# mariaalfaroc/omr_a2s_multimodal_transformer

Hardware: AMD Instinct MI355X
Metric: training samples/sec (higher is better)
Workload: dtype bf16; 1 GPU; C2: image encoder (CNN) + 6-layer d_model=256 kern decoder, fwd+bwd+Adam, dropout on, teacher-forcing noise on; one sample = one score image + its token sequence; per_gpu_batch=32, global_batch=32, image=256x2048x1, seq_len=512, layers=6, d_model=256, vocab=6997, parallelism=dp1

## Files before the change

include/omr_hip.h:

```cpp
#ifndef OMR_HIP_H
#define OMR_HIP_H
#ifdef __cplusplus
extern "C" {
#endif

#define OMR_DTYPE_F32 0
#define OMR_DTYPE_BF16 1
#define OMR_DTYPE_U8 2

int omr_abi_version(void);

int omr_cast(const void* src, int src_dtype, void* dst, int dst_dtype, long n, void* stream);
int omr_add(int dtype, const void* a, const void* b, void* out, long n, void* stream);
int omr_relu_bwd(int dtype, const void* dy, const void* y, void* dx, long n, float scale, void* stream);
int omr_dropout(int dtype, const void* x, void* out, long n, float p, unsigned long long seed, int channel_mode, long per_sample, int C,
                void* stream);
int omr_embed_pe_fwd(int dtype, const long* tokens, const void* table, const float* pe, void* out, long M, int T_len, int d, int vocab,
                     void* stream);
int omr_embed_bwd(int dtype, const long* tokens, const void* dout, float* dtable, long M, int d, int pad_idx, int vocab, void* stream);
int omr_add_pe2d(int dtype, const void* x, const float* pe_hwc, void* out, int B, int h, int w, int C, int maxh, int maxw, void* stream);
int omr_colsum(int dtype, const void* dy, float* db, long M, int N, long ld, void* stream);
int omr_adam(float* p, const float* g, float* m, float* v, void* p_bf16, long n, int step, float lr, float b1, float b2, float eps,
             float grad_scale, void* stream);
int omr_argmax(const float* x, int rows, int n, long ld, long* idx_out, float* val_out, void* stream);
// ... 54 lines not shown
                               const OmrAugment* aug, int dst_dtype, void* out, int B, int H, int W, float pad_value, void* stream);

int omr_gemm(int dtype, int c_dtype, int transA, int transB, int M, int N, int K, const void* A, long lda, const void* B, long ldb, void* C,
             long ldc, const float* bias, int relu, int accumulate, int split_k, float* colsum_a, float drop_p,
             unsigned long long drop_seed, int row_group, int row_group_stride, int row_group_base, int row_group_operand, void* stream);

int omr_quantize_rows_fp8(int dtype, const void* x, long ldx, unsigned char* q, long ldq, float* scale, int M, int K, void* stream);
int omr_gemm_fp8(int c_dtype, int M, int N, int K, const unsigned char* A8, long lda, const float* scale_a, const unsigned char* W8, long ldb,
                 const float* scale_w, void* C, long ldc, const float* bias, int relu, void* stream);

typedef struct omr_dw_problem {
    const void* dy; const void* x; float* dw; float* db;
    int rows, n_out, n_in, row_group; long ld_dy, ld_x, ld_dw; int row_group_stride, row_group_base;
} omr_dw_problem;
int omr_linear_wgrad_grouped(int dtype, int nprob, const omr_dw_problem* problems, void* stream);

int omr_conv3x3_stat_slots(int B, int Ho, int Wo);
int omr_instnorm_reduce_sums(void* workspace, int slots, int B, int C, void* stream);
int omr_conv3x3_fwd(int dtype, const void* x, const void* w, const float* bias, void* y, const float* in_mean, const float* in_rstd,
                    const void* out_mask, float mask_scale, int B, int H, int W, int CIN, int COUT, int stride_h, int stride_w, int dil_h,
                    int dil_w, int Ho, int Wo, int relu, float drop_p, unsigned long long drop_seed, int drop_channel_mode,
                    int stat_mode, double* stat_ws, int stat_slots, const void* stat_x, const float* stat_mean, const float* stat_rstd,
                    void* stream);
int omr_conv3x3_weight_flip(int dtype, const void* w, void* wd, int COUT, int CIN, void* stream);
typedef struct omr_flip_desc { const void* w; void* wd; int cout, cin; } omr_flip_desc;
int omr_conv3x3_weight_flip_grouped(int dtype, int n, const omr_flip_desc* descs, void* stream);
int omr_conv3x3_wgrad(int dtype, const void* x, const void* dy, float* dw, float* db, const float* in_mean, const float* in_rstd, int B, int H, int W,
                      int CIN, int COUT, int stride_h, int stride_w, int Ho, int Wo, void* stream);
int omr_conv3x3_bwd_fused(const void* g, const void* x, const void* w_flipped, void* dx, float* dw, float* db, int B, int H, int W, int CIN,
                          int COUT, int mask_input, float mask_scale, const void* norm_y, const float* norm_mean, const float* norm_rstd,
                          const void* norm_workspace, int norm_slots, int relu_mask, float relu_scale, const float* x_mean, const float* x_rstd,
                          void* stat_workspace, int stat_slots, void* stream);
int omr_conv3x3_bwd_fused_s2(const void* g, const void* x, const void* w_flipped, void* dx, float* dw, float* db, int B, int H, int W,
                             const float* x_mean, const float* x_rstd, void* stat_workspace, int stat_slots, void* stream);
int omr_dwconv3x3(int dtype, const void* x, const void* w, const float* bias, void* y, const float* in_mean, const float* in_rstd,
                  const void* out_mask, float mask_scale, int B, int H, int W, int C, int flip, void* stream);
int omr_dwconv3x3_wgrad(int dtype, const void* x, const void* dy, float* dw, float* db, const float* in_mean, const float* in_rstd, int B,
                        int H, int W, int C, void* stream);

int omr_attn_fwd(int dtype, const void* q, const void* k, const void* v, void* o, float* lse, long ldq, long ldk, long ldv, long ldo,
                 long bsq, long bsk, long bsv, long bso, int B, int H, int T, int S, int head_dim, int causal, int window,
                 const float* key_bias, const int* blk_lq, const int* blk_lkv, float dropout_p, unsigned long long seed,
                 const unsigned long long* drop_words, void* stream);
long omr_attn_dropout_words_count(int B, int H, int T, int S);
int omr_attn_dropout_words(unsigned long long* words, int B, int H, int T, int S, float dropout_p, unsigned long long seed, void* stream);
long omr_attn_workspace_floats(int B, int H, int T, int S, int head_dim, int causal, int backward);
// ... 207 lines not shown
```

omr_a2s_multimodal_transformer_amd/csrc/conv.hip:

```cpp
#include <type_traits>

#include "omr_common.h"
#include "omr_hip.h"

#include "conv3x3_mfma.h"
#include "conv_wgrad.h"
#include "conv1.h"

using omr_conv::ConvArgs;
using omr_conv::TW;
int omr_conv3x3_dispatch_bf16(const ConvArgs& a, hipStream_t s);
int omr_conv3x3_dispatch_f32(const ConvArgs& a, hipStream_t s);

namespace {

constexpr int FLIP_MAX = 32;
struct FlipTable { const void* w[FLIP_MAX]; void* wd[FLIP_MAX]; int cout[FLIP_MAX]; int cin[FLIP_MAX]; };
template <typename T>
__global__ void weight_flip_grouped_kernel(FlipTable t) {
    const int g = blockIdx.y, COUT = t.cout[g], CIN = t.cin[g];
    const T* __restrict__ w = (const T*)t.w[g];
    T* __restrict__ wd = (T*)t.wd[g];
    const long total = (long)COUT * 9 * CIN;
    for (long i = blockIdx.x * (long)blockDim.x + threadIdx.x; i < total; i += (long)gridDim.x * blockDim.x) {
// ... 175 lines not shown
    int gx = (OMR_NUM_CU * occv + gy - 1) / gy; if (gx < 1) gx = 1; if (gx > ntiles) gx = ntiles;
    hipLaunchKernelGGL(kern, dim3(gx, gy), dim3(256), shm, s, a);
    OMR_CHECK_LAUNCH();
    return OMR_OK;
}

template <typename T, int TH, int SH, int SW> int launch_wgrad2(const WgradArgs& a, hipStream_t s) {
    if (a.COUT > 32 && a.CIN > 32) return launch_wgrad3<T, TH, 64, 64, SH, SW>(a, s);
    if (a.COUT > 32) return launch_wgrad3<T, TH, 64, 32, SH, SW>(a, s);
    return launch_wgrad3<T, TH, 32, 32, SH, SW>(a, s);
}

template <typename T, int TH1, int TH2> int launch_wgrad(const WgradArgs& a, hipStream_t s) {
    if (a.sh == 1 && a.sw == 1) return launch_wgrad2<T, TH1, 1, 1>(a, s);
    if (a.sh == 2 && a.sw == 2) return launch_wgrad2<T, TH2, 2, 2>(a, s);
    if (a.sh == 2 && a.sw == 1) return launch_wgrad2<T, TH2, 2, 1>(a, s);
    return OMR_ERR_UNSUPPORTED;
}

inline int ew_grid(long n) { long g = (n + 255) / 256; return (int)(g < 1 ? 1 : (g > 4096 ? 4096 : g)); }

}

extern "C" int omr_conv3x3_fwd(int dtype, const void* x, const void* w, const float* bias, void* y, const float* in_mean, const float* in_rstd,
                               const void* out_mask, float mask_scale, int B, int H, int W, int CIN, int COUT, int stride_h, int stride_w,
                               int dil_h, int dil_w, int Ho, int Wo, int relu, float drop_p, unsigned long long drop_seed,
                               int drop_channel_mode, int stat_mode, double* stat_ws, int stat_slots, const void* stat_x,
                               const float* stat_mean, const float* stat_rstd, void* stream) {
    if (B <= 0 || H <= 0 || W <= 0 || CIN <= 0 || COUT <= 0 || !x || !w || (!y && stat_mode != 4)) return OMR_ERR_ARG;
    if (stride_h < 1 || stride_w < 1 || dil_h < 1 || dil_w < 1 || dil_h > 2 || dil_w > 2) return OMR_ERR_ARG;
    if ((stride_h > 1 || stride_w > 1) && (dil_h > 1 || dil_w > 1)) return OMR_ERR_UNSUPPORTED;
    hipStream_t s = (hipStream_t)stream;
    if (drop_p < 0.f || drop_p >= 1.f || stat_mode < 0 || stat_mode == 3 || stat_mode > 5) return OMR_ERR_ARG;
    if (stat_mode && (!stat_ws || stat_slots < 1)) return OMR_ERR_ARG;
    if (stat_mode >= 2 && (!stat_x || !stat_mean || !stat_rstd)) return OMR_ERR_ARG;
    if (stat_mode >= 4 && (out_mask || bias || drop_p > 0.f)) return OMR_ERR_ARG;
    if (CIN == 1) {
        if (drop_p > 0.f || stat_mode) return OMR_ERR_UNSUPPORTED;
        if (dil_h != 1 || dil_w != 1 || stride_h != 1 || stride_w != 1 || in_mean || out_mask || Ho != H || Wo != W) return OMR_ERR_UNSUPPORTED;
        return omr_conv1_fwd(dtype, x, w, bias, y, B, H, W, COUT, relu, s);
    }
    ConvArgs a;
    a.x = x; a.w = w; a.bias = bias; a.y = y; a.mean = in_mean; a.rstd = in_rstd; a.mask = out_mask; a.mask_scale = mask_scale;
    a.B = B; a.Hr = H; a.Wr = W; a.CIN = CIN; a.Ho = Ho; a.Wo = Wo; a.COUT = COUT;
    a.sh = stride_h; a.sw = stride_w; a.dh = dil_h; a.dw = dil_w; a.relu = relu; a.tiles_w = a.tiles_h = 0;
    a.drop_thresh = OMR_DROP_THRESH16(drop_p); a.drop_scale = 1.f / (1.f - drop_p); a.drop_seed = drop_seed;
    a.drop_channel = drop_channel_mode;
    a.stat_mode = stat_mode; a.stat_ws = stat_ws; a.stat_x = stat_x; a.stat_mean = stat_mean; a.stat_rstd = stat_rstd; a.stat_slots = stat_slots;
    a.stat_relu = 0; a.stat_relu_scale = 1.f;
    if (stat_mode >= 4) { a.stat_relu = relu; a.stat_relu_scale = mask_scale; a.relu = 0; a.mask_scale = 1.f; }
    if (dtype == OMR_BF16) return omr_conv3x3_dispatch_bf16(a, s);
    if (dtype == OMR_F32) return omr_conv3x3_dispatch_f32(a, s);
    return OMR_ERR_UNSUPPORTED;
}

extern "C" int omr_conv3x3_stat_slots(int B, int Ho, int Wo) {
    if (B <= 0 || Ho <= 0 || Wo <= 0) return OMR_ERR_ARG;
    const long tiles = (long)cdiv(Ho, 4) * cdiv(Wo, TW), slots = ((long)OMR_NUM_CU * 8 + B - 1) / B;
    return (int)(tiles < slots ? tiles : slots);
}

extern "C" int omr_conv3x3_weight_flip(int dtype, const void* w, void* wd, int COUT, int CIN, void* stream) {
    if (COUT <= 0 || CIN <= 0) return OMR_ERR_ARG;
    FlipTable t = {};
    t.w[0] = w; t.wd[0] = wd; t.cout[0] = COUT; t.cin[0] = CIN;
    DISPATCH_T(dtype, hipLaunchKernelGGL((weight_flip_grouped_kernel<T>), ew_grid((long)COUT * 9 * CIN), 256, 0, (hipStream_t)stream, t));
    OMR_CHECK_LAUNCH();
    return OMR_OK;
}

extern "C" int omr_conv3x3_weight_flip_grouped(int dtype, int n, const omr_flip_desc* descs, void* stream) {
    if (n < 0 || (n && !descs)) return OMR_ERR_ARG;
// ... 41 lines not shown
```

omr_a2s_multimodal_transformer_amd/csrc/conv3x3_mfma.h:

```cpp
#pragma once
#include <type_traits>

#include "omr_common.h"
#include "launch_setup.h"
#include "instnorm_slots.h"

namespace omr_conv {

constexpr int NORM_MAX = 128;
constexpr int TW = 32;

template <int G, typename F, typename LoadFn, typename StoreFn>
__device__ __forceinline__ void staged_walk(int pix0, int npix, int DP, int il0, int jl0, int di, int dj, int IW, LoadFn load, StoreFn store) {
    int il = il0, jl = jl0;
    for (int base = pix0; base < npix; base += G * DP) {
        F v[G];
        int pix = base;
#pragma unroll
        for (int g = 0; g < G; ++g) {
            if (pix < npix) v[g] = load(il, jl);
            jl += dj; il += di;
            if (jl >= IW) { jl -= IW; ++il; }
            pix += DP;
        }
        pix = base;
#pragma unroll
        for (int g = 0; g < G; ++g) {
            if (pix < npix) store(pix, v[g]);
            pix += DP;
        }
    }
}

__host__ __device__ constexpr bool conv_subpix(int SH, int SW, int DH, int DW, int RPW) { return DH == 2 && DW == 2 && SH == 1 && SW == 1 && RPW == 2; }
__host__ __device__ constexpr int conv_halo_h(int TH, int SH, bool subpix) { return subpix ? ((TH - 1) * SH + 3 + 1) / 2 : (TH - 1) * SH + 3; }
__host__ __device__ constexpr int conv_halo_w(int SW, bool subpix) { return subpix ? ((TW - 1) * SW + 3) / 2 : (TW - 1) * SW + 3; }

struct ConvArgs {
    const void* x; const void* w; const float* bias; void* y;
    const float* mean; const float* rstd;
    const void* mask; float mask_scale;
    int B, Hr, Wr, CIN, Ho, Wo, COUT;
    int sh, sw, dh, dw, relu, tiles_w, tiles_h;
    uint32_t drop_thresh; float drop_scale; uint64_t drop_seed; int drop_channel;
    int stat_mode; double* stat_ws; const void* stat_x; const float* stat_mean; const float* stat_rstd; int stat_slots;
    int stat_relu; float stat_relu_scale;
};

template <typename T, int NT, int RPW, int CK, int SH, int SW, int DH, int DW, bool SINGLE, int EPI>
__global__ __launch_bounds__(256, (SINGLE && NT == 32) ? ((CK == 16 && EPI != 2) ? 4 : 3) : 2) void conv3x3_mfma_kernel(ConvArgs a) {
    typedef typename Frag<T>::type F;
    typedef __attribute__((ext_vector_type(4))) T T4;
    constexpr int VEC = Frag<T>::N;
    constexpr int CKP = CK + VEC;
    constexpr int NB = NT / 32;
    constexpr int TH = 4 * RPW;
    constexpr bool SUBPIX = conv_subpix(SH, SW, DH, DW, RPW);
    constexpr int IH = conv_halo_h(TH, SH, SUBPIX), IW = conv_halo_w(SW, SUBPIX), NPIX = IH * IW;
    constexpr int CPP = CK / VEC;
    constexpr int OP = NT + VEC;
    constexpr int XS_ELEMS = (SINGLE && TH * TW * OP > NPIX * CKP) ? TH * TW * OP : NPIX * CKP;
    extern __shared__ __attribute__((aligned(16))) unsigned char smem_raw[];
    T* Xs = reinterpret_cast<T*>(smem_raw);
    T* Os = Xs;
    T* Ws = Xs + XS_ELEMS;

    const int tid = threadIdx.x, lane = tid & 63, wave = tid >> 6;
    const int n0 = blockIdx.y * NT;
    const int Hv = (a.Hr - 1) * DH + 1, Wv = (a.Wr - 1) * DW + 1;
    const T* W = (const T*)a.w;
    constexpr bool single = SINGLE;
    const int frow = lane & 31, fk = (lane >> 5) * VEC, hsel = 4 * (lane >> 5);
    const int sp_rp = wave >> 1;
    const int sp_row = (wave & 1) * 4 + sp_rp + 2 * (frow >> 4), sp_col = 2 * (frow & 15);

    auto stage_weights = [&](int c0) {
        constexpr int NCH = NT * 9 * CPP, ROUNDS = (NCH + 255) / 256, GB = 4;
#pragma unroll
        for (int r0 = 0; r0 < ROUNDS; r0 += GB) {
            F v[GB];
#pragma unroll
            for (int g = 0; g < GB; ++g) {
                const int c = tid + (r0 + g) * 256, row = c / CPP, kc = (c % CPP) * VEC, n = n0 + row / 9;
                v[g] = frag_zero<T>();
                if (r0 + g < ROUNDS && c < NCH && n < a.COUT) v[g] = *reinterpret_cast<const F*>(W + ((long)n * 9 + row % 9) * a.CIN + c0 + kc);
            }
#pragma unroll
            for (int g = 0; g < GB; ++g) {
                const int c = tid + (r0 + g) * 256, row = c / CPP, kc = (c % CPP) * VEC;
                if (r0 + g < ROUNDS && c < NCH) *reinterpret_cast<F*>(Ws + (long)row * CKP + kc) = v[g];
            }
        }
    };

    __shared__ __attribute__((aligned(16))) float sbias[NT];
    for (int i = tid; i < NT; i += 256) sbias[i] = (a.bias && n0 + i < a.COUT) ? a.bias[n0 + i] : 0.f;

    __shared__ __attribute__((aligned(16))) float snorm[2 * NORM_MAX];
    if (a.mean)
        for (int i = tid; i < a.CIN; i += 256) {
            snorm[i] = a.mean[(long)blockIdx.z * a.CIN + i];
            snorm[NORM_MAX + i] = a.rstd[(long)blockIdx.z * a.CIN + i];
        }

    if (single) stage_weights(0);

    constexpr int CPO = NT / VEC;
    constexpr int NSV = EPI ? VEC : 1;
    float ssum[NSV], ssq[NSV], smu[EPI == 2 ? VEC : 1], srs[EPI == 2 ? VEC : 1];
#pragma unroll
    for (int e = 0; e < NSV; ++e) ssum[e] = ssq[e] = 0.f;
#pragma unroll
    for (int e = 0; e < (EPI == 2 ? VEC : 1); ++e) { smu[e] = 0.f; srs[e] = 1.f; }
    constexpr bool FWD = EPI == 1 || EPI == 3, DROP = EPI == 3;
    const bool stat1 = FWD && a.stat_mode == 1, stat2 = EPI == 2 && (a.stat_mode == 2 || a.stat_mode == 4);
    const bool apply5 = EPI == 2 && a.stat_mode == 5, store_y = a.stat_mode != 4;
    auto flush_stats = [&](int bimg) {
        if constexpr (EPI != 0) {
            constexpr int NGRP = 256 / CPO;
            constexpr int RP = NT + 1;
            static_assert((size_t)NGRP * RP * sizeof(float) <= ((size_t)XS_ELEMS + (size_t)NT * 9 * CKP) * sizeof(T), "reduction scratch fits in the (dead) halo + weight tiles");
            float* red = reinterpret_cast<float*>(smem_raw);
#pragma unroll
            for (int k = 0; k < 2; ++k) {
                __syncthreads();
                const int kcs = (tid % CPO) * VEC, grp = tid / CPO;
#pragma unroll
                for (int e = 0; e < NSV; ++e) red[grp * RP + kcs + e] = k ? ssq[e] : ssum[e];
                __syncthreads();
                for (int i = tid; i < NT; i += 256) {
                    const int n = n0 + i;
                    double acc2 = 0.0;
                    for (int g = 0; g < NGRP; ++g) acc2 += (double)red[g * RP + i];
                    if (n < a.COUT) slot_store(a.stat_ws, bimg, a.stat_slots, a.COUT, n, k, acc2);
                }
            }
        }
    };

    const int tiles_per_img = a.tiles_h * a.tiles_w;
    const int b = blockIdx.z;
    if constexpr (EPI == 2) {
        if (stat2 || apply5) {
            const double* compact = a.stat_ws + slot_compact_offset(a.B, a.stat_slots, a.COUT);
            const double inv_hw = 1.0 / ((double)a.Ho * a.Wo);
#pragma unroll
            for (int e = 0; e < VEC; ++e) {
                const int n = n0 + (tid % CPO) * VEC + e;
                smu[e] = n < a.COUT ? a.stat_mean[(long)b * a.COUT + n] : 0.f;
                srs[e] = n < a.COUT ? a.stat_rstd[(long)b * a.COUT + n] : 1.f;
                if (apply5) {
                    ssum[e] = n < a.COUT ? (float)(compact[((long)b * a.COUT + n) * 2] * inv_hw) : 0.f;
                    ssq[e] = n < a.COUT ? (float)(compact[((long)b * a.COUT + n) * 2 + 1] * inv_hw) : 0.f;
                }
            }
        }
    }
    uint32_t ckeep[NB];
#pragma unroll
    for (int j = 0; j < NB; ++j) ckeep[j] = 0xffffu;
    if constexpr (DROP) {
        if (a.drop_thresh && a.drop_channel) {
#pragma unroll
            for (int j = 0; j < NB; ++j) {
                ckeep[j] = 0;
#pragma unroll
                for (int r = 0; r < 16; r += 2) {
                    const uint32_t hsh = drop_pair_bits(a.drop_seed, ((uint64_t)b * a.COUT + n0 + j * 32 + 8 * (r >> 2) + hsel + (r & 3)) >> 1);
                    ckeep[j] |= (uint32_t)((hsh & 0xffffu) >= a.drop_thresh) << r | (uint32_t)((hsh >> 16) >= a.drop_thresh) << (r + 1);
                }
            }
        }
    }
    constexpr bool PF = true;
    constexpr int XR = (NPIX + 255) / 256;
    constexpr int WNCH = NT * 9 * CPP, WR = SINGLE ? 1 : (WNCH + 255) / 256;
    F xv[XR][CPP], wv[WR];
    unsigned xok = 0;
    const T* X = (const T*)a.x + (long)b * a.Hr * a.Wr * a.CIN;
    auto load_x = [&](int rem, int c0) {
        const int th = rem / a.tiles_w, tw = rem - th * a.tiles_w;
        const int vh0 = th * TH * SH - 1, vw0 = tw * TW * SW - 1;
        xok = 0;
#pragma unroll
        for (int r = 0; r < XR; ++r) {
            const int pix = tid + r * 256;
            const int il = pix / IW, jl = pix - il * IW;
            const int vh = vh0 + (SUBPIX ? 2 * il + 1 : il), vw = vw0 + (SUBPIX ? 2 * jl + 1 : jl);
            const bool ok = pix < NPIX && vh >= 0 && vh < Hv && vw >= 0 && vw < Wv && (vh & (DH - 1)) == 0 && (vw & (DW - 1)) == 0;
            const T* src = X + ((long)(vh >> (DH >> 1)) * a.Wr + (vw >> (DW >> 1))) * a.CIN + c0;
#pragma unroll
            for (int k = 0; k < CPP; ++k) {
                xv[r][k] = frag_zero<T>();
                if (ok) xv[r][k] = *reinterpret_cast<const F*>(src + k * VEC);
            }
            xok |= (unsigned)ok << r;
        }
    };
    auto store_x = [&](int c0) {
#pragma unroll
        for (int r = 0; r < XR; ++r) {
            const int pix = tid + r * 256;
            if (a.mean && ((xok >> r) & 1)) {
#pragma unroll
                for (int k = 0; k < CPP; ++k)
#pragma unroll
                    for (int q4 = 0; q4 < VEC / 4; ++q4) {
                        const f32x4 mu = *reinterpret_cast<const f32x4*>(&snorm[c0 + k * VEC + 4 * q4]);
                        const f32x4 rs = *reinterpret_cast<const f32x4*>(&snorm[NORM_MAX + c0 + k * VEC + 4 * q4]);
#pragma unroll
                        for (int e = 0; e < 4; ++e)
                            xv[r][k][4 * q4 + e] = from_f32<T>((to_f32(xv[r][k][4 * q4 + e]) - mu[e]) * rs[e]);
                    }
            }
            if (pix < NPIX)
#pragma unroll
                for (int k = 0; k < CPP; ++k) *reinterpret_cast<F*>(Xs + (long)pix * CKP + k * VEC) = xv[r][k];
        }
    };
    auto load_w = [&](int c0) {
#pragma unroll
        for (int r = 0; r < WR; ++r) {
            const int c = tid + r * 256, row = c / CPP, kc = (c % CPP) * VEC, n = n0 + row / 9;
            wv[r] = frag_zero<T>();
            if (c < WNCH && n < a.COUT) wv[r] = *reinterpret_cast<const F*>(W + ((long)n * 9 + row % 9) * a.CIN + c0 + kc);
        }
    };
    auto store_w = [&]() {
#pragma unroll
        for (int r = 0; r < WR; ++r) {
            const int c = tid + r * 256, row = c / CPP, kc = (c % CPP) * VEC;
            if (c < WNCH) *reinterpret_cast<F*>(Ws + (long)row * CKP + kc) = wv[r];
        }
    };
    if constexpr (PF) {
        if ((int)blockIdx.x < tiles_per_img) { load_x(blockIdx.x, 0); load_w(0); }
    }

    for (int rem = blockIdx.x; rem < tiles_per_img; rem += gridDim.x) {
        const int th = rem / a.tiles_w, tw = rem - th * a.tiles_w;
        const int oh0 = th * TH, ow0 = tw * TW;
        const int vh0 = oh0 * SH - 1;

        f32x16 acc[RPW][NB];
#pragma unroll
        for (int i = 0; i < RPW; ++i)
#pragma unroll
            for (int j = 0; j < NB; ++j)
#pragma unroll
                for (int r = 0; r < 16; ++r) acc[i][j][r] = 0.f;

        for (int c0 = 0; c0 < a.CIN; c0 += CK) {
            __syncthreads();
            if constexpr (!PF) load_x(rem, c0);
            store_x(c0);
            if constexpr (!SINGLE) store_w();
            __syncthreads();
            if constexpr (PF) {
                int nc0 = c0 + CK, nrem = rem;
                if (nc0 >= a.CIN) { nc0 = 0; nrem = rem + gridDim.x; }
                if (nrem < tiles_per_img) { load_x(nrem, nc0); load_w(nc0); }
            }
            bool row_live[RPW][3];
#pragma unroll
            for (int i = 0; i < RPW; ++i)
#pragma unroll
                for (int kh = 0; kh < 3; ++kh) row_live[i][kh] = DH == 1 || (((vh0 + (wave * RPW + i) * SH + kh) & (DH - 1)) == 0);
            if constexpr (SUBPIX) {
                const int vw0 = ow0 * SW - 1;
#pragma unroll
                for (int tap = 0; tap < 9; ++tap) {
                    const int kh = tap / 3, kw = tap % 3;
                    if (((vh0 + sp_rp + kh) & 1) != 0) continue;
                    const bool lc[2] = {((vw0 + kw) & 1) == 0, ((vw0 + 1 + kw) & 1) == 0};
#pragma unroll
                    for (int kk = 0; kk < CK; kk += KStep<T>::value) {
                        F af[2], bf[NB];
#pragma unroll
                        for (int cp = 0; cp < 2; ++cp)
                            if (lc[cp]) af[cp] = *reinterpret_cast<const F*>(Xs + (long)(((sp_row + kh) >> 1) * IW + ((sp_col + cp + kw) >> 1)) * CKP + kk + fk);
#pragma unroll
                        for (int j = 0; j < NB; ++j)
                            bf[j] = *reinterpret_cast<const F*>(Ws + (long)((j * 32 + frow) * 9 + tap) * CKP + kk + fk);
#pragma unroll
                        for (int cp = 0; cp < 2; ++cp) {
                            if (!lc[cp]) continue;
#pragma unroll
                            for (int j = 0; j < NB; ++j) mma32(acc[cp][j], bf[j], af[cp]);
                        }
                    }
                }
            } else
#pragma unroll
            for (int tap = 0; tap < 9; ++tap) {
                const int kh = tap / 3, kw = tap % 3;
                bool any_live = false;
#pragma unroll
                for (int i = 0; i < RPW; ++i) any_live = any_live || row_live[i][kh];
                if (!any_live) continue;
#pragma unroll
                for (int kk = 0; kk < CK; kk += KStep<T>::value) {
                    F af[RPW], bf[NB];
#pragma unroll
                    for (int i = 0; i < RPW; ++i) {
                        const int pix = ((wave * RPW + i) * SH + kh) * IW + frow * SW + kw;
                        af[i] = *reinterpret_cast<const F*>(Xs + (long)pix * CKP + kk + fk);
                    }
#pragma unroll
                    for (int j = 0; j < NB; ++j)
                        bf[j] = *reinterpret_cast<const F*>(Ws + (long)((j * 32 + frow) * 9 + tap) * CKP + kk + fk);
#pragma unroll
                    for (int i = 0; i < RPW; ++i) {
                        if (!row_live[i][kh]) continue;
#pragma unroll
                        for (int j = 0; j < NB; ++j) mma32(acc[i][j], bf[j], af[i]);
                    }
                }
            }
        }

        const float oscale = a.mask ? a.mask_scale : 1.f;
        const bool drop_chan = DROP && a.drop_thresh != 0 && a.drop_channel;
        __syncthreads();
#pragma unroll
        for (int j = 0; j < NB; ++j)
#pragma unroll
            for (int i = 0; i < RPW; ++i) {
                T* orow = Os + (long)(SUBPIX ? sp_row * TW + sp_col + i : (wave * RPW + i) * TW + frow) * OP + j * 32 + hsel;
#pragma unroll
                for (int g = 0; g < 4; ++g) {
                    T4 o;
                    const uint32_t k4 = ckeep[j] >> (4 * g);
                    const f32x4 bq = *reinterpret_cast<const f32x4*>(&sbias[j * 32 + 8 * g + hsel]);
#pragma unroll
                    for (int e = 0; e < 4; ++e) {
                        float v = acc[i][j][4 * g + e] + bq[e];
                        if (a.relu) v = fmaxf(v, 0.f);
                        if constexpr (DROP) {
                            if (drop_chan) v = ((k4 >> e) & 1u) ? v * a.drop_scale : 0.f;
                        } else {
                            v *= oscale;
                        }
                        o[e] = from_f32<T>(v);
                    }
                    *reinterpret_cast<T4*>(orow + 8 * g) = o;
                }
            }
        __syncthreads();
        T* Y = (T*)a.y + (long)b * a.Ho * a.Wo * a.COUT;
        const T* Mk = a.mask ? (const T*)a.mask + (long)b * a.Ho * a.Wo * a.COUT : nullptr;
        const T* SX = (stat2 || apply5) ? (const T*)a.stat_x + (long)b * a.Ho * a.Wo * a.COUT : nullptr;
#pragma unroll(EPI == 0 ? 8 : 4)
        for (int c = tid; c < TH * TW * CPO; c += 256) {
            const int pl = c / CPO, kc = (c % CPO) * VEC;
            const int oh = oh0 + pl / TW, ow = ow0 + pl % TW, n = n0 + kc;
            if (oh >= a.Ho || ow >= a.Wo || n >= a.COUT) continue;
            F v = *reinterpret_cast<const F*>(Os + (long)pl * OP + kc);
            const long o = ((long)oh * a.Wo + ow) * a.COUT + n;
            if constexpr (DROP) {
                if (a.drop_thresh && !a.drop_channel) {
                    const uint64_t pbase = ((uint64_t)b * a.Ho * a.Wo * a.COUT + (uint64_t)o) >> 1;
                    const uint32_t h0 = (uint32_t)pbase ^ (uint32_t)(pbase >> 32) * 0x27D4EB2Fu;
                    const uint32_t slo = (uint32_t)a.drop_seed, shi = (uint32_t)(a.drop_seed >> 32);
#pragma unroll
                    for (int e = 0; e < VEC / 2; ++e) {
                        const uint32_t hsh = hash32(slo, shi, h0 ^ (uint32_t)e);
                        v[2 * e] = (hsh & 0xffffu) >= a.drop_thresh ? from_f32<T>(to_f32(v[2 * e]) * a.drop_scale) : from_f32<T>(0.f);
                        v[2 * e + 1] = (hsh >> 16) >= a.drop_thresh ? from_f32<T>(to_f32(v[2 * e + 1]) * a.drop_scale) : from_f32<T>(0.f);
                    }
                }
            }
            if (Mk) {
                typedef typename std::conditional<sizeof(T) == 2, short, int>::type I;
                typedef __attribute__((ext_vector_type(VEC))) I IV;
                const IV m = *reinterpret_cast<const IV*>(Mk + o);
                const IV keep = m > (I)0;
// ... 12 lines not shown
                        if (a.stat_relu) d = xf > 0.f ? d * a.stat_relu_scale : 0.f;
                        v[e] = from_f32<T>(d);
                    }
                }
            }
            if (store_y) *reinterpret_cast<F*>(Y + o) = v;
            if constexpr (FWD) {
                if (stat1) {
#pragma unroll
                    for (int e = 0; e < VEC; ++e) { const float f = to_f32(v[e]); ssum[e] += f; ssq[e] += f * f; }
                }
            } else if constexpr (EPI == 2) {
                if (stat2) {
                    const F xv = *reinterpret_cast<const F*>(SX + o);
#pragma unroll
                    for (int e = 0; e < VEC; ++e) { const float f = to_f32(v[e]); ssum[e] += f; ssq[e] += f * ((to_f32(xv[e]) - smu[e]) * srs[e]); }
                }
            }
        }
    }
    if (stat1 || stat2) flush_stats(b);
}

template <typename T, int NT, int RPW, int CK, int SH, int SW, int DH, int DW, bool SINGLE, int EPI> int launch_conv3(const ConvArgs& a0, hipStream_t s) {
    ConvArgs a = a0;
    constexpr int TH = 4 * RPW;
    constexpr int CKP = CK + Frag<T>::N;
    constexpr bool SUBPIX = conv_subpix(SH, SW, DH, DW, RPW);
    constexpr int IH = conv_halo_h(TH, SH, SUBPIX), IW = conv_halo_w(SW, SUBPIX), NPIX = IH * IW, OP = NT + Frag<T>::N;
    constexpr int XS_ELEMS = (SINGLE && TH * TW * OP > NPIX * CKP) ? TH * TW * OP : NPIX * CKP;
    a.tiles_w = cdiv(a.Wo, TW);
    a.tiles_h = cdiv(a.Ho, TH);
    size_t shm = ((size_t)XS_ELEMS + (size_t)NT * 9 * CKP) * sizeof(T);
    if (!SINGLE && (size_t)TH * TW * OP * sizeof(T) > shm) shm = (size_t)TH * TW * OP * sizeof(T);
    if (shm > 160 * 1024) return OMR_ERR_UNSUPPORTED;
    if (a.COUT % Frag<T>::N) return OMR_ERR_UNSUPPORTED;
    if (a.mean && a.CIN > NORM_MAX) return OMR_ERR_UNSUPPORTED;
    auto kern = conv3x3_mfma_kernel<T, NT, RPW, CK, SH, SW, DH, DW, SINGLE, EPI>;
    const int ny = cdiv(a.COUT, NT);
    const long tiles_per_img = (long)a.tiles_w * a.tiles_h;
    static std::atomic<int> occ_cache{0};
    const int occv = omr_launch_setup(occ_cache, (const void*)kern, shm, shm > 48 * 1024, 256, 2);
    if (occv == 0) return OMR_ERR_LAUNCH;
    long gx = ((long)OMR_NUM_CU * occv + (long)ny * a.B - 1) / ((long)ny * a.B);
    if (gx > tiles_per_img) gx = tiles_per_img;
    if (a.stat_mode) {
        if (a.stat_slots < 1) return OMR_ERR_ARG;
        if (gx > a.stat_slots) gx = a.stat_slots;
    }
    if (gx < 1) gx = 1;
    hipLaunchKernelGGL(kern, dim3((unsigned)gx, ny, a.B), dim3(256), shm, s, a);
    OMR_CHECK_LAUNCH();
    return OMR_OK;
}

template <typename T, int NT, int RPW, int CK, int SH, int SW, int DH, int DW, bool SINGLE> int launch_conv2(const ConvArgs& a, hipStream_t s) {
    constexpr bool can1 = (DH == 1 && DW == 1), can2 = (SH == 1 && SW == 1);
    constexpr bool is_f32 = std::is_same<T, float>::value;
    int epi = (a.stat_mode == 2 || a.stat_mode >= 4) ? 2 : (a.drop_thresh ? 3 : (a.stat_mode == 1 ? 1 : 0));
    if (is_f32 && epi == 0) epi = can1 ? 1 : 2;
    if (epi == 1) {
        if constexpr (can1) return launch_conv3<T, NT, RPW, CK, SH, SW, DH, DW, SINGLE, 1>(a, s);
        else return OMR_ERR_UNSUPPORTED;
    }
    if (epi == 3) {
        if constexpr (can1) return launch_conv3<T, NT, RPW, CK, SH, SW, DH, DW, SINGLE, 3>(a, s);
        else return OMR_ERR_UNSUPPORTED;
    }
    if (epi == 2) {
        if constexpr (can2) return launch_conv3<T, NT, RPW, CK, SH, SW, DH, DW, SINGLE, 2>(a, s);
        else return OMR_ERR_UNSUPPORTED;
    }
    if constexpr (!is_f32) return launch_conv3<T, NT, RPW, CK, SH, SW, DH, DW, SINGLE, 0>(a, s);
    else return OMR_ERR_UNSUPPORTED;
}
template <typename T, int NT, int RPW, int CK, int SH, int SW, int DH, int DW> int launch_conv(const ConvArgs& a, hipStream_t s) {
    if (a.CIN == CK) return launch_conv2<T, NT, RPW, CK, SH, SW, DH, DW, true>(a, s);
    return launch_conv2<T, NT, RPW, CK, SH, SW, DH, DW, false>(a, s);
}

template <typename T, int NT, int SH, int SW, int DH, int DW> int dispatch_conv_ck(const ConvArgs& a, hipStream_t s) {
    constexpr int KS = KStep<T>::value;
    constexpr bool strided = SH > 1 || SW > 1;
    if (a.CIN % KS) return OMR_ERR_UNSUPPORTED;
    if constexpr (strided) {
        return launch_conv<T, NT, 1, KS, SH, SW, DH, DW>(a, s);
    } else {
        if (a.CIN % (2 * KS) == 0) return launch_conv<T, NT, 2, 2 * KS, SH, SW, DH, DW>(a, s);
        return launch_conv<T, NT, 2, KS, SH, SW, DH, DW>(a, s);
    }
}
template <typename T, int NT> int dispatch_conv_nt(const ConvArgs& a, hipStream_t s) {
    if (a.dh == 1 && a.dw == 1) {
        if (a.sh == 1 && a.sw == 1) return dispatch_conv_ck<T, NT, 1, 1, 1, 1>(a, s);
        if (a.sh == 2 && a.sw == 2) return dispatch_conv_ck<T, NT, 2, 2, 1, 1>(a, s);
        if (a.sh == 2 && a.sw == 1) return dispatch_conv_ck<T, NT, 2, 1, 1, 1>(a, s);
        return OMR_ERR_UNSUPPORTED;
    }
    if (a.sh != 1 || a.sw != 1) return OMR_ERR_UNSUPPORTED;
    if (a.dh == 2 && a.dw == 2) return dispatch_conv_ck<T, NT, 1, 1, 2, 2>(a, s);
    if (a.dh == 2 && a.dw == 1) return dispatch_conv_ck<T, NT, 1, 1, 2, 1>(a, s);
    return OMR_ERR_UNSUPPORTED;
}
template <typename T> int dispatch_conv(const ConvArgs& a, hipStream_t s) {
    return a.COUT > 32 ? dispatch_conv_nt<T, 64>(a, s) : dispatch_conv_nt<T, 32>(a, s);
}


}
```

omr_a2s_multimodal_transformer_amd/kernels.py:

```python
from __future__ import annotations

import ctypes
import math
from typing import Optional, Tuple

import torch

from ._lib import cur_stream, dtype_code, header_constant, lib, ptr, require_cuda

Tensor = torch.Tensor


def _rows2d(t: Tensor) -> Tuple[int, int, int]:
    assert t.dim() == 2 and t.stride(1) == 1, f"expected a row-major 2-D tensor, got shape {tuple(t.shape)} strides {t.stride()}"
    return t.shape[0], t.shape[1], t.stride(0)


def _omr_gemm(a: Tensor, b: Tensor, out: Tensor, M: int, N: int, K: int, trans_a, trans_b, bias, relu, accumulate, split_k, colsum_a, drop, group) -> Tensor:
    require_cuda(a, b, bias, out, colsum_a)
    assert a.dtype == b.dtype
    lib().call("omr_gemm", dtype_code(a.dtype), dtype_code(out.dtype), int(trans_a), int(trans_b), M, N, K, ptr(a), a.stride(0), ptr(b), b.stride(0),
               ptr(out), out.stride(0), ptr(bias), int(relu), int(accumulate), split_k, ptr(colsum_a), float(drop[0]) if drop else 0.0,
               (int(drop[1]) & (2**64 - 1)) if drop else 0, *group, cur_stream())
    return out
# ... 616 lines not shown
    Ho, Wo = out_hw
    y = torch.empty((B, Ho, Wo, COUT), dtype=x.dtype, device=x.device) if stat_mode != 4 else None
    mean = rstd = None
    if in_stats is not None:
        mean, rstd = in_stats
        assert tuple(mean.shape) == (B, CIN) and mean.dtype == torch.float32
    if out_mask is not None:
        assert tuple(out_mask.shape) == (B, Ho, Wo, COUT) and out_mask.is_contiguous() and out_mask.dtype == x.dtype
    if bias is not None:
        assert bias.dtype == torch.float32 and bias.numel() == COUT
    p, seed, chan = drop if drop is not None else (0.0, 0, False)
    smean = srstd = None
    if stat_mode:
        assert stat_ws is not None and stat_ws.dtype == torch.float64 and stat_slots >= 1 and stat_ws.numel() >= slot_workspace_elems(B, COUT, stat_slots)
    if stat_mode >= 2:
        smean, srstd = stat_stats
        assert stat_x is not None and tuple(stat_x.shape) == (B, Ho, Wo, COUT) and stat_x.is_contiguous() and tuple(smean.shape) == (B, COUT)
    lib().call("omr_conv3x3_fwd", dtype_code(x.dtype), ptr(x), ptr(w_phys), ptr(bias), ptr(y), ptr(mean), ptr(rstd), ptr(out_mask), float(mask_scale),
               B, H, W, CIN, COUT, stride[0], stride[1], dil[0], dil[1], Ho, Wo, int(relu), float(p), int(seed) & (2**64 - 1), int(chan),
               int(stat_mode), ptr(stat_ws), int(stat_slots), ptr(stat_x), ptr(smean), ptr(srstd), cur_stream())
    return y


def instnorm_reduce_sums(ws: Tensor, slots: int, B: int, C: int) -> None:
    require_cuda(ws)
    lib().call("omr_instnorm_reduce_sums", ptr(ws), slots, B, C, cur_stream())


def conv3x3_weight_flip(w_phys: Tensor) -> Tensor:
    require_cuda(w_phys)
    COUT, _, _, CIN = w_phys.shape
    wd = torch.empty((CIN, 3, 3, COUT), dtype=w_phys.dtype, device=w_phys.device)
    lib().call("omr_conv3x3_weight_flip", dtype_code(w_phys.dtype), ptr(w_phys), ptr(wd), COUT, CIN, cur_stream())
    return wd


class _FlipDesc(ctypes.Structure):
    _fields_ = [("w", ctypes.c_void_p), ("wd", ctypes.c_void_p), ("cout", ctypes.c_int), ("cin", ctypes.c_int)]


def conv3x3_weight_flip_table(pairs):
    arr = (_FlipDesc * len(pairs))()
    dt = pairs[0][0].dtype
    for q, (w, wd) in zip(arr, pairs):
        require_cuda(w, wd)
        COUT, _, _, CIN = w.shape
# ... 500 lines not shown
```

Before: 1400 samples/s.

## Add 8-wave tall and wide workgroup variants to the MFMA 3x3 conv

```diff
diff --git a/include/omr_hip.h b/include/omr_hip.h
--- a/include/omr_hip.h
+++ b/include/omr_hip.h
@@ -100,6 +100,8 @@
                     int dil_w, int Ho, int Wo, int relu, float drop_p, unsigned long long drop_seed, int drop_channel_mode,
                     int stat_mode, double* stat_ws, int stat_slots, const void* stat_x, const float* stat_mean, const float* stat_rstd,
                     void* stream);
+int omr_conv3x3_set_route(int route);
+int omr_conv3x3_route(int B, int CIN, int COUT, int Ho, int Wo, int epilogue);
 int omr_conv3x3_weight_flip(int dtype, const void* w, void* wd, int COUT, int CIN, void* stream);
 typedef struct omr_flip_desc { const void* w; void* wd; int cout, cin; } omr_flip_desc;
 int omr_conv3x3_weight_flip_grouped(int dtype, int n, const omr_flip_desc* descs, void* stream);
diff --git a/omr_a2s_multimodal_transformer_amd/csrc/conv.hip b/omr_a2s_multimodal_transformer_amd/csrc/conv.hip
--- a/omr_a2s_multimodal_transformer_amd/csrc/conv.hip
+++ b/omr_a2s_multimodal_transformer_amd/csrc/conv.hip
@@ -221,6 +221,25 @@
 
 }
 
+static std::atomic<int> g_conv_route{-1};
+
+extern "C" int omr_conv3x3_set_route(int route) {
+    if (route < -1 || route > omr_conv::CONV_WIDE) return OMR_ERR_ARG;
+    g_conv_route.store(route, std::memory_order_relaxed);
+    return OMR_OK;
+}
+
+extern "C" int omr_conv3x3_route(int B, int CIN, int COUT, int Ho, int Wo, int epilogue) {
+    if (B <= 0 || CIN <= 0 || COUT <= 0 || Ho <= 0 || Wo <= 0 || epilogue < 0 || epilogue > 3) return OMR_ERR_ARG;
+    if (COUT <= 32 || CIN % 32) return omr_conv::CONV_WG4;
+    ConvArgs a = {};
+    a.B = B; a.CIN = CIN; a.COUT = COUT; a.Ho = Ho; a.Wo = Wo;
+    a.stat_mode = epilogue == 2 ? 2 : (epilogue ? 1 : 0); a.drop_thresh = epilogue == 3;
+    a.route = g_conv_route.load(std::memory_order_relaxed);
+    const int wg = omr_conv::conv_route(a, 32);
+    return wg < 0 ? OMR_ERR_UNSUPPORTED : wg;
+}
+
 extern "C" int omr_conv3x3_fwd(int dtype, const void* x, const void* w, const float* bias, void* y, const float* in_mean, const float* in_rstd,
                                const void* out_mask, float mask_scale, int B, int H, int W, int CIN, int COUT, int stride_h, int stride_w,
                                int dil_h, int dil_w, int Ho, int Wo, int relu, float drop_p, unsigned long long drop_seed,
@@ -247,6 +266,7 @@
     a.drop_channel = drop_channel_mode;
     a.stat_mode = stat_mode; a.stat_ws = stat_ws; a.stat_x = stat_x; a.stat_mean = stat_mean; a.stat_rstd = stat_rstd; a.stat_slots = stat_slots;
     a.stat_relu = 0; a.stat_relu_scale = 1.f;
+    a.route = g_conv_route.load(std::memory_order_relaxed);
     if (stat_mode >= 4) { a.stat_relu = relu; a.stat_relu_scale = mask_scale; a.relu = 0; a.mask_scale = 1.f; }
     if (dtype == OMR_BF16) return omr_conv3x3_dispatch_bf16(a, s);
     if (dtype == OMR_F32) return omr_conv3x3_dispatch_f32(a, s);
diff --git a/omr_a2s_multimodal_transformer_amd/csrc/conv3x3_mfma.h b/omr_a2s_multimodal_transformer_amd/csrc/conv3x3_mfma.h
--- a/omr_a2s_multimodal_transformer_amd/csrc/conv3x3_mfma.h
+++ b/omr_a2s_multimodal_transformer_amd/csrc/conv3x3_mfma.h
@@ -35,6 +35,11 @@
 __host__ __device__ constexpr bool conv_subpix(int SH, int SW, int DH, int DW, int RPW) { return DH == 2 && DW == 2 && SH == 1 && SW == 1 && RPW == 2; }
 __host__ __device__ constexpr int conv_halo_h(int TH, int SH, bool subpix) { return subpix ? ((TH - 1) * SH + 3 + 1) / 2 : (TH - 1) * SH + 3; }
 __host__ __device__ constexpr int conv_halo_w(int SW, bool subpix) { return subpix ? ((TW - 1) * SW + 3) / 2 : (TW - 1) * SW + 3; }
+
+enum { CONV_WG4 = 0, CONV_TALL = 1, CONV_WIDE = 2 };
+__host__ __device__ constexpr int conv_threads(int WG) { return WG == CONV_WG4 ? 256 : 512; }
+__host__ __device__ constexpr int conv_tile_h(int RPW, int WG) { return (WG == CONV_TALL ? 8 : 4) * RPW; }
+__host__ __device__ constexpr int conv_block_couts(int NT, int WG) { return WG == CONV_WIDE ? 2 * NT : NT; }
 
 struct ConvArgs {
     const void* x; const void* w; const float* bias; void* y;
@@ -45,20 +50,24 @@
     uint32_t drop_thresh; float drop_scale; uint64_t drop_seed; int drop_channel;
     int stat_mode; double* stat_ws; const void* stat_x; const float* stat_mean; const float* stat_rstd; int stat_slots;
     int stat_relu; float stat_relu_scale;
+    int route;
 };
 
-template <typename T, int NT, int RPW, int CK, int SH, int SW, int DH, int DW, bool SINGLE, int EPI>
-__global__ __launch_bounds__(256, (SINGLE && NT == 32) ? ((CK == 16 && EPI != 2) ? 4 : 3) : 2) void conv3x3_mfma_kernel(ConvArgs a) {
+template <typename T, int NT, int RPW, int CK, int SH, int SW, int DH, int DW, bool SINGLE, int EPI, int WG = CONV_WG4>
+__global__ __launch_bounds__(conv_threads(WG), (SINGLE && NT == 32) ? ((CK == 16 && EPI != 2) ? 4 : 3) : 2) void conv3x3_mfma_kernel(ConvArgs a) {
     typedef typename Frag<T>::type F;
     typedef __attribute__((ext_vector_type(4))) T T4;
     constexpr int VEC = Frag<T>::N;
     constexpr int CKP = CK + VEC;
     constexpr int NB = NT / 32;
-    constexpr int TH = 4 * RPW;
+    constexpr int NTHR = conv_threads(WG);
+    constexpr int BNT = conv_block_couts(NT, WG);
+    constexpr int TH = conv_tile_h(RPW, WG);
     constexpr bool SUBPIX = conv_subpix(SH, SW, DH, DW, RPW);
+    static_assert(WG == CONV_WG4 || (!SUBPIX && NT == 64), "8-wave workgroups: 64 couts per wave, no sub-pixel row mapping");
     constexpr int IH = conv_halo_h(TH, SH, SUBPIX), IW = conv_halo_w(SW, SUBPIX), NPIX = IH * IW;
     constexpr int CPP = CK / VEC;
-    constexpr int OP = NT + VEC;
+    constexpr int OP = BNT + VEC;
     constexpr int XS_ELEMS = (SINGLE && TH * TW * OP > NPIX * CKP) ? TH * TW * OP : NPIX * CKP;
     extern __shared__ __attribute__((aligned(16))) unsigned char smem_raw[];
     T* Xs = reinterpret_cast<T*>(smem_raw);
@@ -66,7 +75,9 @@
     T* Ws = Xs + XS_ELEMS;
 
     const int tid = threadIdx.x, lane = tid & 63, wave = tid >> 6;
-    const int n0 = blockIdx.y * NT;
+    const int wrow = WG == CONV_WIDE ? (wave & 3) : wave;
+    const int wn = WG == CONV_WIDE ? (wave >> 2) * NT : 0;
+    const int n0 = blockIdx.y * BNT;
     const int Hv = (a.Hr - 1) * DH + 1, Wv = (a.Wr - 1) * DW + 1;
     const T* W = (const T*)a.w;
     constexpr bool single = SINGLE;
@@ -75,37 +86,37 @@
     const int sp_row = (wave & 1) * 4 + sp_rp + 2 * (frow >> 4), sp_col = 2 * (frow & 15);
 
     auto stage_weights = [&](int c0) {
-        constexpr int NCH = NT * 9 * CPP, ROUNDS = (NCH + 255) / 256, GB = 4;
+        constexpr int NCH = BNT * 9 * CPP, ROUNDS = (NCH + NTHR - 1) / NTHR, GB = 4;
 #pragma unroll
         for (int r0 = 0; r0 < ROUNDS; r0 += GB) {
             F v[GB];
 #pragma unroll
             for (int g = 0; g < GB; ++g) {
-                const int c = tid + (r0 + g) * 256, row = c / CPP, kc = (c % CPP) * VEC, n = n0 + row / 9;
+                const int c = tid + (r0 + g) * NTHR, row = c / CPP, kc = (c % CPP) * VEC, n = n0 + row / 9;
                 v[g] = frag_zero<T>();
                 if (r0 + g < ROUNDS && c < NCH && n < a.COUT) v[g] = *reinterpret_cast<const F*>(W + ((long)n * 9 + row % 9) * a.CIN + c0 + kc);
             }
 #pragma unroll
             for (int g = 0; g < GB; ++g) {
-                const int c = tid + (r0 + g) * 256, row = c / CPP, kc = (c % CPP) * VEC;
+                const int c = tid + (r0 + g) * NTHR, row = c / CPP, kc = (c % CPP) * VEC;
                 if (r0 + g < ROUNDS && c < NCH) *reinterpret_cast<F*>(Ws + (long)row * CKP + kc) = v[g];
             }
         }
     };
 
-    __shared__ __attribute__((aligned(16))) float sbias[NT];
-    for (int i = tid; i < NT; i += 256) sbias[i] = (a.bias && n0 + i < a.COUT) ? a.bias[n0 + i] : 0.f;
+    __shared__ __attribute__((aligned(16))) float sbias[BNT];
+    for (int i = tid; i < BNT; i += NTHR) sbias[i] = (a.bias && n0 + i < a.COUT) ? a.bias[n0 + i] : 0.f;
 
     __shared__ __attribute__((aligned(16))) float snorm[2 * NORM_MAX];
     if (a.mean)
-        for (int i = tid; i < a.CIN; i += 256) {
+        for (int i = tid; i < a.CIN; i += NTHR) {
             snorm[i] = a.mean[(long)blockIdx.z * a.CIN + i];
             snorm[NORM_MAX + i] = a.rstd[(long)blockIdx.z * a.CIN + i];
         }
 
     if (single) stage_weights(0);
 
-    constexpr int CPO = NT / VEC;
+    constexpr int CPO = BNT / VEC;
     constexpr int NSV = EPI ? VEC : 1;
     float ssum[NSV], ssq[NSV], smu[EPI == 2 ? VEC : 1], srs[EPI == 2 ? VEC : 1];
 #pragma unroll
@@ -117,9 +128,9 @@
     const bool apply5 = EPI == 2 && a.stat_mode == 5, store_y = a.stat_mode != 4;
     auto flush_stats = [&](int bimg) {
         if constexpr (EPI != 0) {
-            constexpr int NGRP = 256 / CPO;
-            constexpr int RP = NT + 1;
-            static_assert((size_t)NGRP * RP * sizeof(float) <= ((size_t)XS_ELEMS + (size_t)NT * 9 * CKP) * sizeof(T), "reduction scratch fits in the (dead) halo + weight tiles");
+            constexpr int NGRP = NTHR / CPO;
+            constexpr int RP = BNT + 1;
+            static_assert((size_t)NGRP * RP * sizeof(float) <= ((size_t)XS_ELEMS + (size_t)BNT * 9 * CKP) * sizeof(T), "reduction scratch fits in the (dead) halo + weight tiles");
             float* red = reinterpret_cast<float*>(smem_raw);
 #pragma unroll
             for (int k = 0; k < 2; ++k) {
@@ -128,7 +139,7 @@
 #pragma unroll
                 for (int e = 0; e < NSV; ++e) red[grp * RP + kcs + e] = k ? ssq[e] : ssum[e];
                 __syncthreads();
-                for (int i = tid; i < NT; i += 256) {
+                for (int i = tid; i < BNT; i += NTHR) {
                     const int n = n0 + i;
                     double acc2 = 0.0;
                     for (int g = 0; g < NGRP; ++g) acc2 += (double)red[g * RP + i];
@@ -166,15 +177,15 @@
                 ckeep[j] = 0;
 #pragma unroll
                 for (int r = 0; r < 16; r += 2) {
-                    const uint32_t hsh = drop_pair_bits(a.drop_seed, ((uint64_t)b * a.COUT + n0 + j * 32 + 8 * (r >> 2) + hsel + (r & 3)) >> 1);
+                    const uint32_t hsh = drop_pair_bits(a.drop_seed, ((uint64_t)b * a.COUT + n0 + wn + j * 32 + 8 * (r >> 2) + hsel + (r & 3)) >> 1);
                     ckeep[j] |= (uint32_t)((hsh & 0xffffu) >= a.drop_thresh) << r | (uint32_t)((hsh >> 16) >= a.drop_thresh) << (r + 1);
                 }
             }
         }
     }
     constexpr bool PF = true;
-    constexpr int XR = (NPIX + 255) / 256;
-    constexpr int WNCH = NT * 9 * CPP, WR = SINGLE ? 1 : (WNCH + 255) / 256;
+    constexpr int XR = (NPIX + NTHR - 1) / NTHR;
+    constexpr int WNCH = BNT * 9 * CPP, WR = SINGLE ? 1 : (WNCH + NTHR - 1) / NTHR;
     F xv[XR][CPP], wv[WR];
     unsigned xok = 0;
     const T* X = (const T*)a.x + (long)b * a.Hr * a.Wr * a.CIN;
@@ -184,7 +195,7 @@
         xok = 0;
 #pragma unroll
         for (int r = 0; r < XR; ++r) {
-            const int pix = tid + r * 256;
+            const int pix = tid + r * NTHR;
             const int il = pix / IW, jl = pix - il * IW;
             const int vh = vh0 + (SUBPIX ? 2 * il + 1 : il), vw = vw0 + (SUBPIX ? 2 * jl + 1 : jl);
             const bool ok = pix < NPIX && vh >= 0 && vh < Hv && vw >= 0 && vw < Wv && (vh & (DH - 1)) == 0 && (vw & (DW - 1)) == 0;
@@ -200,7 +211,7 @@
     auto store_x = [&](int c0) {
 #pragma unroll
         for (int r = 0; r < XR; ++r) {
-            const int pix = tid + r * 256;
+            const int pix = tid + r * NTHR;
             if (a.mean && ((xok >> r) & 1)) {
 #pragma unroll
                 for (int k = 0; k < CPP; ++k)
@@ -221,7 +232,7 @@
     auto load_w = [&](int c0) {
 #pragma unroll
         for (int r = 0; r < WR; ++r) {
-            const int c = tid + r * 256, row = c / CPP, kc = (c % CPP) * VEC, n = n0 + row / 9;
+            const int c = tid + r * NTHR, row = c / CPP, kc = (c % CPP) * VEC, n = n0 + row / 9;
             wv[r] = frag_zero<T>();
             if (c < WNCH && n < a.COUT) wv[r] = *reinterpret_cast<const F*>(W + ((long)n * 9 + row % 9) * a.CIN + c0 + kc);
         }
@@ -229,7 +240,7 @@
     auto store_w = [&]() {
 #pragma unroll
         for (int r = 0; r < WR; ++r) {
-            const int c = tid + r * 256, row = c / CPP, kc = (c % CPP) * VEC;
+            const int c = tid + r * NTHR, row = c / CPP, kc = (c % CPP) * VEC;
             if (c < WNCH) *reinterpret_cast<F*>(Ws + (long)row * CKP + kc) = wv[r];
         }
     };
@@ -265,7 +276,7 @@
 #pragma unroll
             for (int i = 0; i < RPW; ++i)
 #pragma unroll
-                for (int kh = 0; kh < 3; ++kh) row_live[i][kh] = DH == 1 || (((vh0 + (wave * RPW + i) * SH + kh) & (DH - 1)) == 0);
+                for (int kh = 0; kh < 3; ++kh) row_live[i][kh] = DH == 1 || (((vh0 + (wrow * RPW + i) * SH + kh) & (DH - 1)) == 0);
             if constexpr (SUBPIX) {
                 const int vw0 = ow0 * SW - 1;
 #pragma unroll
@@ -303,12 +314,12 @@
                     F af[RPW], bf[NB];
 #pragma unroll
                     for (int i = 0; i < RPW; ++i) {
-                        const int pix = ((wave * RPW + i) * SH + kh) * IW + frow * SW + kw;
+                        const int pix = ((wrow * RPW + i) * SH + kh) * IW + frow * SW + kw;
                         af[i] = *reinterpret_cast<const F*>(Xs + (long)pix * CKP + kk + fk);
                     }
 #pragma unroll
                     for (int j = 0; j < NB; ++j)
-                        bf[j] = *reinterpret_cast<const F*>(Ws + (long)((j * 32 + frow) * 9 + tap) * CKP + kk + fk);
+                        bf[j] = *reinterpret_cast<const F*>(Ws + (long)((wn + j * 32 + frow) * 9 + tap) * CKP + kk + fk);
 #pragma unroll
                     for (int i = 0; i < RPW; ++i) {
                         if (!row_live[i][kh]) continue;
@@ -326,12 +337,12 @@
         for (int j = 0; j < NB; ++j)
 #pragma unroll
             for (int i = 0; i < RPW; ++i) {
-                T* orow = Os + (long)(SUBPIX ? sp_row * TW + sp_col + i : (wave * RPW + i) * TW + frow) * OP + j * 32 + hsel;
+                T* orow = Os + (long)(SUBPIX ? sp_row * TW + sp_col + i : (wrow * RPW + i) * TW + frow) * OP + wn + j * 32 + hsel;
 #pragma unroll
                 for (int g = 0; g < 4; ++g) {
                     T4 o;
                     const uint32_t k4 = ckeep[j] >> (4 * g);
-                    const f32x4 bq = *reinterpret_cast<const f32x4*>(&sbias[j * 32 + 8 * g + hsel]);
+                    const f32x4 bq = *reinterpret_cast<const f32x4*>(&sbias[wn + j * 32 + 8 * g + hsel]);
 #pragma unroll
                     for (int e = 0; e < 4; ++e) {
                         float v = acc[i][j][4 * g + e] + bq[e];
@@ -351,7 +362,7 @@
         const T* Mk = a.mask ? (const T*)a.mask + (long)b * a.Ho * a.Wo * a.COUT : nullptr;
         const T* SX = (stat2 || apply5) ? (const T*)a.stat_x + (long)b * a.Ho * a.Wo * a.COUT : nullptr;
 #pragma unroll(EPI == 0 ? 8 : 4)
-        for (int c = tid; c < TH * TW * CPO; c += 256) {
+        for (int c = tid; c < TH * TW * CPO; c += NTHR) {
             const int pl = c / CPO, kc = (c % CPO) * VEC;
             const int oh = oh0 + pl / TW, ow = ow0 + pl % TW, n = n0 + kc;
             if (oh >= a.Ho || ow >= a.Wo || n >= a.COUT) continue;
@@ -410,25 +421,25 @@
     if (stat1 || stat2) flush_stats(b);
 }
 
-template <typename T, int NT, int RPW, int CK, int SH, int SW, int DH, int DW, bool SINGLE, int EPI> int launch_conv3(const ConvArgs& a0, hipStream_t s) {
+template <typename T, int NT, int RPW, int CK, int SH, int SW, int DH, int DW, bool SINGLE, int EPI, int WG = CONV_WG4> int launch_conv3(const ConvArgs& a0, hipStream_t s) {
     ConvArgs a = a0;
-    constexpr int TH = 4 * RPW;
+    constexpr int TH = conv_tile_h(RPW, WG), NTHR = conv_threads(WG), BNT = conv_block_couts(NT, WG);
     constexpr int CKP = CK + Frag<T>::N;
     constexpr bool SUBPIX = conv_subpix(SH, SW, DH, DW, RPW);
-    constexpr int IH = conv_halo_h(TH, SH, SUBPIX), IW = conv_halo_w(SW, SUBPIX), NPIX = IH * IW, OP = NT + Frag<T>::N;
+    constexpr int IH = conv_halo_h(TH, SH, SUBPIX), IW = conv_halo_w(SW, SUBPIX), NPIX = IH * IW, OP = BNT + Frag<T>::N;
     constexpr int XS_ELEMS = (SINGLE && TH * TW * OP > NPIX * CKP) ? TH * TW * OP : NPIX * CKP;
     a.tiles_w = cdiv(a.Wo, TW);
     a.tiles_h = cdiv(a.Ho, TH);
-    size_t shm = ((size_t)XS_ELEMS + (size_t)NT * 9 * CKP) * sizeof(T);
+    size_t shm = ((size_t)XS_ELEMS + (size_t)BNT * 9 * CKP) * sizeof(T);
     if (!SINGLE && (size_t)TH * TW * OP * sizeof(T) > shm) shm = (size_t)TH * TW * OP * sizeof(T);
     if (shm > 160 * 1024) return OMR_ERR_UNSUPPORTED;
     if (a.COUT % Frag<T>::N) return OMR_ERR_UNSUPPORTED;
     if (a.mean && a.CIN > NORM_MAX) return OMR_ERR_UNSUPPORTED;
-    auto kern = conv3x3_mfma_kernel<T, NT, RPW, CK, SH, SW, DH, DW, SINGLE, EPI>;
-    const int ny = cdiv(a.COUT, NT);
+    auto kern = conv3x3_mfma_kernel<T, NT, RPW, CK, SH, SW, DH, DW, SINGLE, EPI, WG>;
+    const int ny = cdiv(a.COUT, BNT);
     const long tiles_per_img = (long)a.tiles_w * a.tiles_h;
     static std::atomic<int> occ_cache{0};
-    const int occv = omr_launch_setup(occ_cache, (const void*)kern, shm, shm > 48 * 1024, 256, 2);
+    const int occv = omr_launch_setup(occ_cache, (const void*)kern, shm, shm > 48 * 1024, NTHR, WG == CONV_WG4 ? 2 : 1);
     if (occv == 0) return OMR_ERR_LAUNCH;
     long gx = ((long)OMR_NUM_CU * occv + (long)ny * a.B - 1) / ((long)ny * a.B);
     if (gx > tiles_per_img) gx = tiles_per_img;
@@ -437,34 +448,49 @@
         if (gx > a.stat_slots) gx = a.stat_slots;
     }
     if (gx < 1) gx = 1;
-    hipLaunchKernelGGL(kern, dim3((unsigned)gx, ny, a.B), dim3(256), shm, s, a);
+    hipLaunchKernelGGL(kern, dim3((unsigned)gx, ny, a.B), dim3(NTHR), shm, s, a);
     OMR_CHECK_LAUNCH();
     return OMR_OK;
 }
 
-template <typename T, int NT, int RPW, int CK, int SH, int SW, int DH, int DW, bool SINGLE> int launch_conv2(const ConvArgs& a, hipStream_t s) {
+inline int conv_epi(const ConvArgs& a) { return (a.stat_mode == 2 || a.stat_mode >= 4) ? 2 : (a.drop_thresh ? 3 : (a.stat_mode == 1 ? 1 : 0)); }
+template <typename T, int NT, int RPW, int CK, int SH, int SW, int DH, int DW, bool SINGLE, int WG = CONV_WG4> int launch_conv2(const ConvArgs& a, hipStream_t s) {
     constexpr bool can1 = (DH == 1 && DW == 1), can2 = (SH == 1 && SW == 1);
     constexpr bool is_f32 = std::is_same<T, float>::value;
-    int epi = (a.stat_mode == 2 || a.stat_mode >= 4) ? 2 : (a.drop_thresh ? 3 : (a.stat_mode == 1 ? 1 : 0));
+    int epi = conv_epi(a);
     if (is_f32 && epi == 0) epi = can1 ? 1 : 2;
     if (epi == 1) {
-        if constexpr (can1) return launch_conv3<T, NT, RPW, CK, SH, SW, DH, DW, SINGLE, 1>(a, s);
+        if constexpr (can1) return launch_conv3<T, NT, RPW, CK, SH, SW, DH, DW, SINGLE, 1, WG>(a, s);
         else return OMR_ERR_UNSUPPORTED;
     }
     if (epi == 3) {
-        if constexpr (can1) return launch_conv3<T, NT, RPW, CK, SH, SW, DH, DW, SINGLE, 3>(a, s);
+        if constexpr (can1) return launch_conv3<T, NT, RPW, CK, SH, SW, DH, DW, SINGLE, 3, WG>(a, s);
         else return OMR_ERR_UNSUPPORTED;
     }
     if (epi == 2) {
-        if constexpr (can2) return launch_conv3<T, NT, RPW, CK, SH, SW, DH, DW, SINGLE, 2>(a, s);
+        if constexpr (can2) return launch_conv3<T, NT, RPW, CK, SH, SW, DH, DW, SINGLE, 2, WG>(a, s);
         else return OMR_ERR_UNSUPPORTED;
     }
-    if constexpr (!is_f32) return launch_conv3<T, NT, RPW, CK, SH, SW, DH, DW, SINGLE, 0>(a, s);
+    if constexpr (!is_f32) return launch_conv3<T, NT, RPW, CK, SH, SW, DH, DW, SINGLE, 0, WG>(a, s);
     else return OMR_ERR_UNSUPPORTED;
 }
-template <typename T, int NT, int RPW, int CK, int SH, int SW, int DH, int DW> int launch_conv(const ConvArgs& a, hipStream_t s) {
-    if (a.CIN == CK) return launch_conv2<T, NT, RPW, CK, SH, SW, DH, DW, true>(a, s);
-    return launch_conv2<T, NT, RPW, CK, SH, SW, DH, DW, false>(a, s);
+template <typename T, int NT, int RPW, int CK, int SH, int SW, int DH, int DW, int WG = CONV_WG4> int launch_conv(const ConvArgs& a, hipStream_t s) {
+    if (a.CIN == CK) return launch_conv2<T, NT, RPW, CK, SH, SW, DH, DW, true, WG>(a, s);
+    return launch_conv2<T, NT, RPW, CK, SH, SW, DH, DW, false, WG>(a, s);
+}
+
+inline bool conv_route_covers(const ConvArgs& a, int wg, int CK) {
+    if (wg == CONV_TALL) return a.COUT <= 64;
+    if (wg == CONV_WIDE) return a.COUT > 64 && a.COUT <= 128 && a.CIN > CK;
+    return wg == CONV_WG4;
+}
+inline int conv_route_auto(const ConvArgs& a) {
+    if (a.CIN == 32 && a.COUT <= 64 && (long)a.B * cdiv(a.Ho, conv_tile_h(2, CONV_TALL)) * cdiv(a.Wo, TW) >= OMR_NUM_CU) return CONV_TALL;
+    return CONV_WG4;
+}
+inline int conv_route(const ConvArgs& a, int CK) {
+    if (a.route < 0) return conv_route_auto(a);
+    return conv_route_covers(a, a.route, CK) ? a.route : -1;
 }
 
 template <typename T, int NT, int SH, int SW, int DH, int DW> int dispatch_conv_ck(const ConvArgs& a, hipStream_t s) {
@@ -474,7 +500,15 @@
     if constexpr (strided) {
         return launch_conv<T, NT, 1, KS, SH, SW, DH, DW>(a, s);
     } else {
-        if (a.CIN % (2 * KS) == 0) return launch_conv<T, NT, 2, 2 * KS, SH, SW, DH, DW>(a, s);
+        if (a.CIN % (2 * KS) == 0) {
+            if constexpr (NT == 64 && DH == 1 && DW == 1 && std::is_same<T, bf16>::value) {
+                const int wg = conv_route(a, 2 * KS);
+                if (wg < 0) return OMR_ERR_UNSUPPORTED;
+                if (wg == CONV_TALL) return launch_conv<T, NT, 2, 2 * KS, SH, SW, DH, DW, CONV_TALL>(a, s);
+                if (wg == CONV_WIDE) return launch_conv2<T, NT, 2, 2 * KS, SH, SW, DH, DW, false, CONV_WIDE>(a, s);
+            }
+            return launch_conv<T, NT, 2, 2 * KS, SH, SW, DH, DW>(a, s);
+        }
         return launch_conv<T, NT, 2, KS, SH, SW, DH, DW>(a, s);
     }
 }
diff --git a/omr_a2s_multimodal_transformer_amd/kernels.py b/omr_a2s_multimodal_transformer_amd/kernels.py
--- a/omr_a2s_multimodal_transformer_amd/kernels.py
+++ b/omr_a2s_multimodal_transformer_amd/kernels.py
@@ -662,6 +662,20 @@
     return y
 
 
+CONV_ROUTES = {"auto": -1, "wg4": 0, "tall": 1, "wide": 2}
+
+
+def conv3x3_set_route(route) -> None:
+    lib().call("omr_conv3x3_set_route", CONV_ROUTES[route] if isinstance(route, str) else int(route))
+
+
+def conv3x3_route(B: int, cin: int, cout: int, Ho: int, Wo: int, epilogue: int = 0) -> int:
+    r = lib().query("omr_conv3x3_route", B, cin, cout, Ho, Wo, epilogue)
+    if r < 0:
+        raise RuntimeError(f"libomr_hip: omr_conv3x3_route failed: {r}")
+    return r
+
+
 def instnorm_reduce_sums(ws: Tensor, slots: int, B: int, C: int) -> None:
     require_cuda(ws)
     lib().call("omr_instnorm_reduce_sums", ptr(ws), slots, B, C, cur_stream())
```

New measurement: 1391 samples/s. No clear change (-0.6%).
